# Ycblue/TransMIL-DeepGraft

Hardware: AMD Instinct MI355X
Metric: slides/sec (fwd+bwd) at N=8192 patches, d=512 (higher is better)
Workload: dtype bf16; 1 GPU; TransMIL_feat 2-class, 1 bag N=8192x512 per GPU, train step fwd+CE+bwd+allreduce+Lookahead(RAdam); execution=hipGraph replay of the whole step (one graph per resident bag), global_batch=1, seq_len=8192, parallelism=dp1, accumulate_grad_batches=1

## Files before the change

transmil_deepgraft_amd/csrc/nystrom.hip:

```cpp
#include <algorithm>
#include "common.h"
#include "nystrom_common.h"
#include "../../include/transmil_hip.h"

namespace {

template <typename T>
__global__ __launch_bounds__(256) void landmarks_kernel(const T* __restrict__ q, const T* __restrict__ k, int n,
                                                        int l, float* __restrict__ ql, float* __restrict__ kl,
                                                        T* __restrict__ ql_t, T* __restrict__ kl_t) {
  const int bh = blockIdx.x, tid = threadIdx.x, tq = tid & 3, o = ((tid >> 2) & 7) * 8;
  const int j = blockIdx.y * 8 + (tid >> 5);
  const int per = (l + 3) / 4, t0 = tq * per, t1 = min(l, t0 + per);
  const T* qp = q + ((size_t)bh * n + (size_t)j * l) * DH + o;
  const T* kp = k + ((size_t)bh * n + (size_t)j * l) * DH + o;
  float sq[8] = {0.f, 0.f, 0.f, 0.f, 0.f, 0.f, 0.f, 0.f}, sk[8] = {0.f, 0.f, 0.f, 0.f, 0.f, 0.f, 0.f, 0.f};
  for (int t = t0; t < t1; t += 9) {
    vec8<T> a[9], b[9];
#pragma unroll
    for (int u = 0; u < 9; ++u) {
      const int tt = min(t + u, t1 - 1);
      a[u] = load8(qp + (size_t)tt * DH);
      b[u] = load8(kp + (size_t)tt * DH);
    }
// ... 373 lines not shown
  float* po = work;
  float* pm = po + (size_t)nkb * nbh * NL * DH;
  float* pl = pm + (size_t)nkb * nbh * NL;
  tm_allow_smem(a3_fwd_kernel, FWD_F32_SMEM);
  a3_fwd_kernel<<<dim3(nkb, nbh, 2), 256, FWD_F32_SMEM, st>>>(ql, (const float*)k, (const float*)v, n, po, pm, pl);
  TM_CHECK_LAUNCH();
  a3_combine_kernel<<<dim3(nbh, NL / 16), 256, 0, st>>>(po, pm, pl, nkb, nbh, w, lse3);
  TM_CHECK_LAUNCH();
  return 0;
}

extern "C" int tm_nys_a3_fwd_sim2(const float* ql, const float* kl, const void* k, const void* v, int nbh, int n,
                                  float* work, float* a2, void* a2s, void* stream) {
  TM_REQUIRE(n > 0 && n % NL == 0, "a3_fwd_sim2: n must be a positive multiple of 256");
  TM_REQUIRE(ql && kl && k && v && work && a2 && a2s, "a3_fwd_sim2: null operand");
  launch_a3_fwd_v2(ql, k, v, nbh, n, work, Sim2Out{kl, a2, (bf16*)a2s}, (hipStream_t)stream);
  TM_CHECK_LAUNCH();
  return 0;
}

extern "C" int tm_nys_a1_fwd(int dtype, const void* q, const void* v, const void* kl_t, const void* y_t,
                             const float* wconv, int nbh, int nh, int n, void* merged, float* lse1, void* stream) {
  TM_REQUIRE(n > 0 && n % NL == 0 && nbh % nh == 0, "a1_fwd: bad shape");
  hipStream_t st = (hipStream_t)stream;
  if (dtype == TM_BF16) {
    const int cph = n / 32;
    int wpg = std::max(1, std::min(tm_cu_count() / std::max(nbh, 1), cph));
    wpg = std::max(wpg, (cph + A1P_MAXCH - 1) / A1P_MAXCH);
    auto kern = a1_fwd_bf16_kernel<false>;
#ifdef TM_DIAG
    if (NYS_SEL == NYS_STAMP_A1_FWD) kern = a1_fwd_bf16_kernel<true>;
#endif
    tm_allow_smem(kern, A1P_BYTES);
    kern<<<dim3(wpg, nbh), 256, A1P_BYTES, st>>>((const bf16*)q, (const bf16*)v, (const bf16*)kl_t,
                                                               (const bf16*)y_t, wconv, n, nh, wpg, (bf16*)merged,
                                                               lse1);
    TM_CHECK_LAUNCH();
    return 0;
  }
  TM_REQUIRE_F32(dtype);
  constexpr size_t sm = FWD_F32_SMEM > A1_EPI_BYTES ? FWD_F32_SMEM : A1_EPI_BYTES;
  tm_allow_smem(a1_fwd_kernel, sm);
  a1_fwd_kernel<<<dim3(n / 128, nbh), 256, sm, st>>>((const float*)q, (const float*)v, (const float*)kl_t,
                                                     (const float*)y_t, wconv, n, nh, (float*)merged, lse1);
  TM_CHECK_LAUNCH();
  return 0;
}

extern "C" int tm_cast_f32(int dtype, const float* x, void* y, long long count, void* stream) {
  if (count == 0) return 0;
  TM_REQUIRE(((uintptr_t)x % 16) == 0 && ((uintptr_t)y % 16) == 0, "cast_f32: 16-B aligned buffers");
  TM_DTYPE_DISPATCH(dtype, (cast_rows_kernel<T><<<(unsigned)((count + 2047) / 2048), 256, 0, (hipStream_t)stream>>>(
                               x, (T*)y, count)));
  TM_CHECK_LAUNCH();
  return 0;
}

extern "C" long long tm_nys_conv_bwd_workspace(int nbags, int nh, int n) {
  const int r = conv_bwd_rows(nbags * nh, n);
  const long long blocks = std::max((n + 63) / 64, (n + r - 1) / r);
  return (long long)nbags * blocks * nh * TAPS * (long long)sizeof(float);
}

extern "C" int tm_nys_conv_bwd(int dtype, const void* dmerged, const void* merged, const void* v, const float* wconv,
                               int nbh, int nh, int n, void* dv, float* d1, float* work, float* dwconv,
                               tm_reduce_queue* rq, void* stream) {
  TM_REQUIRE(nbh % nh == 0 && n > 0, "conv_bwd: bad shape");
  hipStream_t st = (hipStream_t)stream;
  if (dtype == TM_BF16) {
    const int r = conv_bwd_rows(nbh, n), nblk = (n + r - 1) / r;
    tm_allow_smem(conv_bwd_mfma_kernel, CbLay::BYTES);
    conv_bwd_mfma_kernel<<<dim3(nblk, nbh), 512, CbLay::BYTES, st>>>(
        (const bf16*)dmerged, (const bf16*)merged, (const bf16*)v, wconv, n, nh, r, (bf16*)dv, d1, work);
    TM_CHECK_LAUNCH();
    return tm_splitk_reduce(work, dwconv, (nbh / nh) * nblk, (long long)nh * TAPS, 1.0f, 0, rq, stream);
  }
  TM_REQUIRE_F32(dtype);
  const int ntb = (n + 63) / 64;
  conv_bwd_kernel<<<dim3(ntb, nbh), 256, 0, st>>>((const float*)dmerged, (const float*)merged, (const float*)v, wconv,
                                                  n, nh, (float*)dv, d1, work);
  TM_CHECK_LAUNCH();
  return tm_splitk_reduce(work, dwconv, (nbh / nh) * ntb, (long long)nh * TAPS, 1.0f, 0, rq, stream);
}

namespace {
int a1_bwd_split(int nbh, int n) {
  const int cph = n / 32;
  const int w = std::min(cph, std::max(1, tm_cu_count() / std::max(nbh, 1)));
  return std::max(w, (cph + BwdLay16::MAXQ / 32 - 1) / (BwdLay16::MAXQ / 32));
}
}

extern "C" long long tm_nys_a1_bwd_workspace(int nbh, int n, int queries_per_wg) {
  const long long slabs = std::max((long long)(n / queries_per_wg), (long long)a1_bwd_split(nbh, n));
  return 2LL * slabs * nbh * NL * DH * (long long)sizeof(float);
}

namespace {
int a1_bwd_impl(int dtype, const void* q, const void* dmerged, const void* kl_t, const void* y_t, const float* lse1,
                const float* d1, int nbh, int nh, int n, int queries_per_wg, float* dq, void* dqkv, float dq_scale,
                float* work, float* dkl, float* dy, int accumulate, tm_reduce_queue* rq, void* stream);
}

extern "C" int tm_nys_a1_bwd(int dtype, const void* q, const void* dmerged, const void* kl_t, const void* y_t,
                             const float* lse1, const float* d1, int nbh, int nh, int n, int queries_per_wg,
                             float* dq, float* work, float* dkl, float* dy, int accumulate, tm_reduce_queue* rq,
                             void* stream) {
  return a1_bwd_impl(dtype, q, dmerged, kl_t, y_t, lse1, d1, nbh, nh, n, queries_per_wg, dq, nullptr, 0.f, work, dkl,
                     dy, accumulate, rq, stream);
}

extern "C" int tm_nys_a1_bwd_dqkv(const void* q, const void* dmerged, const void* kl_t, const void* y_t,
                                  const float* lse1, const float* d1, int nbh, int nh, int n, void* dqkv,
                                  float dq_scale, float* work, float* dkl, float* dy, tm_reduce_queue* rq,
                                  void* stream) {
  TM_REQUIRE(dqkv && ((uintptr_t)dqkv % 16) == 0 && nbh % nh == 0, "a1_bwd_dqkv: dqkv");
  return a1_bwd_impl(TM_BF16, q, dmerged, kl_t, y_t, lse1, d1, nbh, nh, n, 256, nullptr, dqkv, dq_scale, work, dkl,
                     dy, 0, rq, stream);
}

namespace {
int a1_bwd_impl(int dtype, const void* q, const void* dmerged, const void* kl_t, const void* y_t, const float* lse1,
                const float* d1, int nbh, int nh, int n, int queries_per_wg, float* dq, void* dqkv, float dq_scale,
                float* work, float* dkl, float* dy, int accumulate, tm_reduce_queue* rq, void* stream) {
  TM_REQUIRE(queries_per_wg % 32 == 0 && n % queries_per_wg == 0, "a1_bwd: queries_per_wg must divide n, x32");
  TM_REQUIRE(dtype != TM_BF16 || queries_per_wg <= NL, "a1_bwd: queries_per_wg must be <= 256 in bf16 mode");
  const bool split = dtype == TM_BF16;
  TM_REQUIRE(!dqkv || split, "a1_bwd_dqkv: the bf16 split kernel only");
  const int nqc = split ? a1_bwd_split(nbh, n) : n / queries_per_wg;
  BwdArgs a{};
  a.q = q; a.q_bag = (long long)nh * n * DH; a.q_head = (long long)n * DH; a.q_row = DH;
  a.dO = dmerged; a.o_bag = (long long)n * nh * DH; a.o_head = DH; a.o_row = nh * DH;
  a.k = kl_t; a.k_bag = (long long)nh * NL * DH; a.k_head = (long long)NL * DH;
  a.v = y_t; a.v_bag = a.k_bag; a.v_head = a.k_head;
  a.lse = lse1; a.lse_bh = n; a.dd = d1; a.dd_bh = n;
  a.dq = dq; a.dq_bh = (long long)n * DH;
  a.dqkv = dqkv; a.dq_scale = dq_scale;
  float* slab_k = work;
  float* slab_v = work + (size_t)nqc * nbh * NL * DH;
  a.dk = slab_k; a.dk_bh = (long long)NL * DH;
  a.dv = slab_v; a.dv_bh = (long long)NL * DH;
  a.slab_stride = (long long)nbh * NL * DH;
  a.nh = nh; a.n_queries_per_wg = queries_per_wg; a.n_key_rows = NL;
  hipStream_t st = (hipStream_t)stream;
  if (split) {
    a.q_total = n;
    a.slab_bf16 = 1;
    auto kern = attn_bwd_bf16_kernel<MODE_A1>;
#ifdef TM_DIAG
    if (NYS_SEL == NYS_STAMP_A1_BWD) kern = attn_bwd_bf16_kernel<MODE_A1, 8, 1>;
    if (NYS_SEL == NYS_STAMP_A1_BWD_CHUNK) kern = attn_bwd_bf16_kernel<MODE_A1, 8, 2>;
#endif
    tm_allow_smem(kern, BwdLay16::BYTES);
    kern<<<dim3(nqc, nbh), 512, BwdLay16::BYTES, st>>>(a);
  } else {
    TM_REQUIRE_F32(dtype);
    tm_allow_smem(attn_bwd_kernel<MODE_A1>, BwdLayF32::BYTES);
    attn_bwd_kernel<MODE_A1><<<dim3(nqc, nbh), 512, BwdLayF32::BYTES, st>>>(a);
  }
  TM_CHECK_LAUNCH();
  const long long cnt = (long long)nbh * NL * DH;
  const int sdt = a.slab_bf16 ? TM_BF16 : TM_F32;
  int rc = tm_splitk_reduce_typed(slab_k, sdt, dkl, nqc, cnt, 1.0f, accumulate, rq, stream);
  if (rc) return rc;
  return tm_splitk_reduce_typed(slab_v, sdt, dy, nqc, cnt, 1.0f, 0, rq, stream);
}
}

namespace {
struct A3Split { int wpg, nw; };
A3Split a3_bwd_split(int nbh, int n) {
  const int units = n / 32;
  const int w = std::max(1, std::min(units, tm_cu_count() / std::max(nbh, 1)));
  const int per = (units + w - 1) / w;
  if (per <= 8) return {w, 8};
  if (per == 9) return {w, 9};
  return {(units + 7) / 8, 8};
}

void launch_a3_bwd_bf16(BwdArgs& a, int nbh, int n, hipStream_t st, int& slabs) {
  const A3Split sp = a3_bwd_split(nbh, n);
  a.q_total = n;
  slabs = sp.wpg;
  if (sp.nw == 9) {
    auto kern = attn_bwd_bf16_kernel<MODE_A3, 9>;
#ifdef TM_DIAG
    if (NYS_SEL == NYS_STAMP_A3_BWD) kern = attn_bwd_bf16_kernel<MODE_A3, 9, 1>;
    if (NYS_SEL == NYS_STAMP_A3_BWD_CHUNK) kern = attn_bwd_bf16_kernel<MODE_A3, 9, 2>;
#endif
    tm_allow_smem(kern, BwdLay9::BYTES);
    kern<<<dim3(sp.wpg, nbh), 576, BwdLay9::BYTES, st>>>(a);
  } else {
    tm_allow_smem(attn_bwd_bf16_kernel<MODE_A3, 8>, BwdLay16::BYTES);
    attn_bwd_bf16_kernel<MODE_A3, 8><<<dim3(sp.wpg, nbh), 512, BwdLay16::BYTES, st>>>(a);
  }
}
}

extern "C" long long tm_nys_a3_bwd_workspace(int nbh, int n) {
  const long long slabs = std::max((long long)(n / NL), (long long)a3_bwd_split(nbh, n).wpg);
  return slabs * nbh * NL * DH * (long long)sizeof(float);
}

extern "C" int tm_nys_a3_bwd(int dtype, const void* ql_t, const void* dw_t, const void* k, const void* v,
                             const float* lse3, const float* d3, int nbh, int nh, int n, float* dk, float* dv,
                             float* work, float* dql, int accumulate, tm_reduce_queue* rq, void* stream) {
  TM_REQUIRE(n % NL == 0, "a3_bwd: n must be a multiple of 256");
  const int nkb = n / NL;
  BwdArgs a{};
  a.q = ql_t; a.q_bag = (long long)nh * NL * DH; a.q_head = (long long)NL * DH; a.q_row = DH;
  a.dO = dw_t; a.o_bag = a.q_bag; a.o_head = a.q_head; a.o_row = DH;
  a.k = k; a.k_bag = (long long)nh * n * DH; a.k_head = (long long)n * DH;
  a.v = v; a.v_bag = a.k_bag; a.v_head = a.k_head;
  a.lse = lse3; a.lse_bh = NL; a.dd = d3; a.dd2 = d3 + (size_t)nbh * NL; a.dd_bh = NL;
  a.dq = work; a.dq_bh = (long long)NL * DH;
  a.slab_stride = (long long)nbh * NL * DH;
  a.dk = dk; a.dk_bh = (long long)n * DH;
  a.dv = dv; a.dv_bh = (long long)n * DH;
  a.nh = nh; a.n_queries_per_wg = NL; a.n_key_rows = n;
  hipStream_t st = (hipStream_t)stream;
  int slabs = nkb;
  if (dtype == TM_BF16) {
    launch_a3_bwd_bf16(a, nbh, n, st, slabs);
  } else {
    TM_REQUIRE_F32(dtype);
    tm_allow_smem(attn_bwd_kernel<MODE_A3>, BwdLayF32::BYTES);
    attn_bwd_kernel<MODE_A3><<<dim3(nkb, nbh), 512, BwdLayF32::BYTES, st>>>(a);
  }
  TM_CHECK_LAUNCH();
  return tm_splitk_reduce(work, dql, slabs, (long long)nbh * NL * DH, 1.0f, accumulate, rq, stream);
}

extern "C" int tm_nys_a3_bwd_fused(const void* ql_t, const void* dw_t, const void* k, const void* v,
                                   const float* lse3, const float* d3, int nbh, int nh, int n, const void* dv_conv,
                                   int dv_lo, int dv_hi, const float* dkl, float* work, float* dql, void* dqkv,
                                   tm_reduce_queue* rq, void* stream) {
  TM_REQUIRE(n % NL == 0 && nbh % nh == 0, "a3_bwd_fused: n must be a multiple of 256");
  TM_REQUIRE(dv_conv && dkl && dqkv, "a3_bwd_fused: null operand");
  const int nkb = n / NL;
  BwdArgs a{};
  a.q = ql_t; a.q_bag = (long long)nh * NL * DH; a.q_head = (long long)NL * DH; a.q_row = DH;
  a.dO = dw_t; a.o_bag = a.q_bag; a.o_head = a.q_head; a.o_row = DH;
  a.k = k; a.k_bag = (long long)nh * n * DH; a.k_head = (long long)n * DH;
  a.v = v; a.v_bag = a.k_bag; a.v_head = a.k_head;
  a.lse = lse3; a.lse_bh = NL; a.dd = d3; a.dd2 = d3 + (size_t)nbh * NL; a.dd_bh = NL;
  a.dq = work; a.dq_bh = (long long)NL * DH;
  a.slab_stride = (long long)nbh * NL * DH;
  a.dv = (float*)dv_conv; a.dv_bh = (long long)n * DH;
  a.nh = nh; a.n_queries_per_wg = NL; a.n_key_rows = n;
  a.dqkv = dqkv; a.dkl = dkl; a.l = n / NL; a.inv_l = 1.0f / (float)(n / NL);
  a.dv_lo = dv_lo; a.dv_hi = dv_hi;
  hipStream_t st = (hipStream_t)stream;
  int slabs = nkb;
  a.slab_bf16 = 1;
  launch_a3_bwd_bf16(a, nbh, n, st, slabs);
  TM_CHECK_LAUNCH();
  if (!dql) return 0;
  return tm_splitk_reduce_typed(work, TM_BF16, dql, slabs, (long long)nbh * NL * DH, 1.0f, 0, rq, stream);
}

extern "C" int tm_nys_a3_bwd_slabs(int nbh, int n) { return a3_bwd_split(nbh, n).wpg; }

extern "C" int tm_nys_assemble_q_slab(int dtype, const float* dq, int dq_row, const float* dql, const void* slab,
                                      int slabs, int nbags, int nh, int n, float scale, void* dqkv, void* stream) {
  TM_REQUIRE(n > 0 && n % NL == 0 && nh > 0 && nh <= 8 && slabs > 0, "assemble_q_slab: bad shape");
  TM_REQUIRE(dq && dql && slab && dqkv, "assemble_q_slab: null operand");
  TM_DTYPE_DISPATCH(dtype, (assemble_q_slab_kernel<T><<<dim3(NL, nbags), AQ_THREADS, 0, (hipStream_t)stream>>>(
                               dq, dq_row, dql, (const bf16*)slab, slabs, (long long)nbags * nh * NL * DH, n, n / NL,
                               nh, scale, (T*)dqkv)));
  TM_CHECK_LAUNCH();
  return 0;
}

extern "C" int tm_nys_assemble_q_slab_inplace(const float* dql, const void* slab, int slabs, int nbags, int nh, int n,
                                              float scale, void* dqkv, void* stream) {
  TM_REQUIRE(n > 0 && n % NL == 0 && nh > 0 && nh <= 8 && slabs > 0, "assemble_q_slab_inplace: bad shape");
  TM_REQUIRE(dql && slab && dqkv && ((uintptr_t)dqkv % 16) == 0, "assemble_q_slab_inplace: null / misaligned operand");
  assemble_q_slab_kernel<bf16, true><<<dim3(NL, nbags), AQ_THREADS, 0, (hipStream_t)stream>>>(
      nullptr, -1, dql, (const bf16*)slab, slabs, (long long)nbags * nh * NL * DH, n, n / NL, nh, scale, (bf16*)dqkv);
  TM_CHECK_LAUNCH();
  return 0;
}

extern "C" int tm_nys_assemble_dqkv(int dtype, const float* dq, const float* dql, const float* dk, const float* dkl,
                                    const float* dv, int nbags, int nh, int n, float scale, void* dqkv,
                                    void* stream) {
  TM_REQUIRE(n % NL == 0, "assemble_dqkv: n must be a multiple of 256");
  const long long items = (long long)n * 3 * nh * DH / 8;
  TM_DTYPE_DISPATCH(dtype, (assemble_dqkv_kernel<T><<<dim3((unsigned)((items + 255) / 256), nbags), 256, 0,
                                                       (hipStream_t)stream>>>(
                               dq, dql, dk, dkl, dv, n, n / NL, nh, scale, (T*)dqkv)));
  TM_CHECK_LAUNCH();
  return 0;
}
```

transmil_deepgraft_amd/csrc/nystrom_bf16.h:

```cpp
#pragma once
#include <algorithm>
#include <type_traits>
#include "nystrom_common.h"
#include "a3_combine.h"

namespace {

constexpr int A1P_WAVES = 4;
constexpr int A1P_MAXCH = 9;
constexpr int A1P_WROWS = A1P_MAXCH * 32 + 32;
constexpr int A1P_OROW = DH + 8;
constexpr size_t A1P_KS = (size_t)NL * Lay<bf16>::KROW * 2;
constexpr size_t A1P_VT = (size_t)NL * Lay<bf16>::VROW * 2;
constexpr size_t A1P_WIN = (size_t)A1P_WROWS * DH * 2;
constexpr size_t A1P_OST = (size_t)32 * A1P_OROW * 2;
constexpr size_t A1P_WIN_OFF = A1P_KS + A1P_VT;
constexpr size_t A1P_OST_OFF = A1P_WIN_OFF + A1P_WIN;
constexpr size_t A1P_BAND_OFF = A1P_OST_OFF + A1P_WAVES * A1P_OST;
constexpr size_t A1P_TAPS_OFF = A1P_BAND_OFF + 4 * 64 * 16;
constexpr size_t A1P_BYTES = A1P_TAPS_OFF + 128 * sizeof(float);

__device__ unsigned long long g_a1_stamps[512 * 8 * 8];
template <bool STAMP>
TM_DEV void a1p_stamp(int slot, int wave) {
// ... 420 lines not shown
  const int k = kb + 8 * (g >> 1) + q;
  typedef __attribute__((address_space(3))) bf16x4 lds_v4;
  const bf16x4 lo = __builtin_amdgcn_ds_read_tr16_b64_v4bf16((lds_v4*)(S + k * ldr + m));
  const bf16x4 hi = __builtin_amdgcn_ds_read_tr16_b64_v4bf16((lds_v4*)(S + (k + 4) * ldr + m));
  return (bf16x8){lo[0], lo[1], lo[2], lo[3], hi[0], hi[1], hi[2], hi[3]};
}

__global__ __launch_bounds__(512) void conv_bwd_mfma_kernel(const bf16* __restrict__ dmerged,
                                                            const bf16* __restrict__ merged,
                                                            const bf16* __restrict__ v,
                                                            const float* __restrict__ wconv, int n, int nh, int R,
                                                            bf16* __restrict__ dv, float* __restrict__ d1,
                                                            float* __restrict__ dw_part) {
  extern __shared__ __attribute__((aligned(16))) char smem[];
  bf16* dos = (bf16*)(smem + CbLay::DO_OFF);
  bf16* vws = (bf16*)(smem + CbLay::V_OFF);
  float* ws = (float*)(smem + CbLay::W_OFF);
  float* csum = (float*)(smem + CbLay::CS_OFF);
  const int tid = threadIdx.x, lane = tid & 63, wave = tid >> 6, r32 = lane & 31, h = lane >> 5;
  const int bh = blockIdx.y, blk = blockIdx.x, nblk = gridDim.x;
  const int head = bh % nh, bag = bh / nh, ld = nh * DH;
  const int t0 = blk * R;
  const int rows = min(R, n - t0);
  const bf16* dob = dmerged + (size_t)bag * n * ld + head * DH;
  const bf16* ob = merged + (size_t)bag * n * ld + head * DH;
  const bf16* vb = v + (size_t)bh * n * DH;
  constexpr int PW = CB_WIN * 8 / 512;
  bf16x8 ca[PW], cb[PW];
#pragma unroll
  for (int j = 0; j < PW; ++j) {
    const int i = tid + 512 * j, w = i >> 3, d0 = (i & 7) * 8, t = t0 - HALF + w;
    const bool ok = t >= 0 && t < n && w < rows + 2 * HALF;
    const int tc = ok ? t : 0;
    ca[j] = load8(dob + (size_t)tc * ld + d0);
    cb[j] = load8(vb + (size_t)tc * DH + d0);
    if (!ok) { ca[j] = (bf16x8){}; cb[j] = (bf16x8){}; }
  }
  if (tid < TAPS) ws[tid] = wconv[head * TAPS + tid];
#pragma unroll
  for (int j = 0; j < PW; ++j) {
    const int i = tid + 512 * j, w = i >> 3, d0 = (i & 7) * 8;
    *(bf16x8*)(dos + w * CB_ROW + d0) = ca[j];
    *(bf16x8*)(vws + w * CB_ROW + d0) = cb[j];
  }
  __syncthreads();
  bf16x8 th[4], tl[4];
#pragma unroll
  for (int st = 0; st < 4; ++st) {
#pragma unroll
    for (int j = 0; j < 8; ++j) {
      const int tau = r32 + 32 - (16 * st + 8 * h + j);
      const float wv = (tau >= 0 && tau < TAPS) ? ws[tau] : 0.f;
      const bf16 hi = (bf16)wv;
      th[st][j] = hi;
      tl[st][j] = (bf16)(wv - (float)hi);
    }
  }
  float* stg = (float*)(smem + CbLay::ST_OFF) + wave * 32 * CB_ST;
  constexpr int NTK = (TAPS + 1) / 2;
  float csl[NTK];
#pragma unroll
  for (int k = 0; k < NTK; ++k) csl[k] = 0.f;
  const int ntile = (rows + 31) / 32;
#pragma unroll 1
  for (int i = wave; i < ntile; i += 8) {
    f32x16 sa = (f32x16){}, sb = (f32x16){};
#pragma unroll
    for (int st = 0; st < 4; ++st) {
      const bf16x8 a = *(const bf16x8*)(dos + (32 * i + HALF + r32) * CB_ROW + 16 * st + 8 * h);
      const bf16x8 ba = *(const bf16x8*)(vws + (32 * i + r32) * CB_ROW + 16 * st + 8 * h);
      const bf16x8 bb = *(const bf16x8*)(vws + (32 * i + 32 + r32) * CB_ROW + 16 * st + 8 * h);
      mma16(sa, a, ba);
      mma16(sb, a, bb);
    }
#pragma unroll
    for (int reg = 0; reg < 16; ++reg) {
      const int row = acc_row(reg, h);
      stg[row * CB_ST + r32] = sa[reg];
      stg[row * CB_ST + 32 + r32] = sb[reg];
    }
    __builtin_amdgcn_fence(__ATOMIC_RELEASE, "wavefront");
    __builtin_amdgcn_wave_barrier();
    __builtin_amdgcn_fence(__ATOMIC_ACQUIRE, "wavefront");
    const int lr = 32 * i + r32;
    const bool rv = lr < rows;
    float wc = 0.f, dd = 0.f;
#pragma unroll
    for (int k = 0; k < NTK; ++k) {
      const int tau = h + 2 * k;
      if (tau < TAPS) {
        const float c = stg[r32 * CB_ST + r32 + tau];
        if (rv) { csl[k] += c; wc = fmaf(ws[tau], c, wc); }
      }
    }
    if (rv) {
      const bf16* orow = ob + (size_t)(t0 + lr) * ld + 32 * h;
      const bf16* grow = dos + (lr + HALF) * CB_ROW + 32 * h;
#pragma unroll
      for (int q = 0; q < 4; ++q) {
        const bf16x8 o8 = load8(orow + 8 * q), g8 = *(const bf16x8*)(grow + 8 * q);
#pragma unroll
        for (int e = 0; e < 8; ++e) dd = fmaf((float)g8[e], (float)o8[e], dd);
      }
    }
    float tot = dd - wc;
    tot += __shfl_xor(tot, 32, 64);
    if (rv && h == 0) d1[(size_t)bh * n + t0 + lr] = tot;
    const bf16* dwin = dos + 32 * i * CB_ROW;
#pragma unroll
    for (int dt = 0; dt < 2; ++dt) {
      f32x16 acc = (f32x16){};
#pragma unroll
      for (int st = 0; st < 4; ++st) {
        const bf16x8 b = frag_tr_rows(dwin, CB_ROW, dt * 32, 16 * st, lane);
        mma16(acc, th[st], b);
        mma16(acc, tl[st], b);
      }
#pragma unroll
      for (int reg = 0; reg < 16; ++reg) {
        const int l2 = 32 * i + acc_row(reg, h);
        if (l2 < rows) dv[((size_t)bh * n + t0 + l2) * DH + dt * 32 + r32] = (bf16)acc[reg];
      }
    }
    __builtin_amdgcn_wave_barrier();
  }
#pragma unroll
  for (int k = 0; k < NTK; ++k) {
    float x = csl[k];
#pragma unroll
    for (int o = 1; o < 32; o <<= 1) x += __shfl_xor(x, o, 64);
    const int tau = h + 2 * k;
    if (r32 == 0 && tau < TAPS) csum[wave * 36 + tau] = x;
  }
  __syncthreads();
  if (tid < TAPS) {
    float sum = 0.f;
#pragma unroll
    for (int w = 0; w < 8; ++w) sum += csum[w * 36 + tid];
    dw_part[((size_t)bag * nblk + blk) * (nh * TAPS) + head * TAPS + tid] = sum;
  }
}

enum NysSel { NYS_AUTO = 0, NYS_STAMP_A1_FWD, NYS_STAMP_A3_FWD, NYS_STAMP_A1_BWD, NYS_STAMP_A1_BWD_CHUNK,
              NYS_STAMP_A3_BWD, NYS_STAMP_A3_BWD_CHUNK };
#ifdef TM_DIAG
int g_nys_sel = NYS_AUTO;
#endif
#define NYS_SEL TM_DIAG_VAR(g_nys_sel)

template <int NW, int MQ>
struct BwdLayT {
  static constexpr int MAXQ = MQ;
  static constexpr int NK = 32 * NW;
  static constexpr int KT_ROW = NK + 8, DS_ROW = NK + 8, QROW = DH + 8;
  static constexpr size_t KT_OFF = 0;
  static constexpr size_t DS_OFF = KT_OFF + DH * KT_ROW * 2;
  static constexpr size_t QS_OFF = DS_OFF + 32 * DS_ROW * 2;
  static constexpr size_t OS_OFF = QS_OFF + MAXQ * QROW * 2;
  static constexpr size_t XC_OFF = OS_OFF + MAXQ * QROW * 2;
  static constexpr size_t LS_OFF = XC_OFF + 6 * 1024 * 4;
  static constexpr size_t MAIN = LS_OFF + 2 * MAXQ * 4;
  static constexpr size_t EPI = (size_t)NK * 68 * 4;
  static constexpr size_t BYTES = MAIN > EPI ? MAIN : EPI;
};
using BwdLay16 = BwdLayT<8, 288>;
using BwdLay9 = BwdLayT<9, 256>;
static_assert(BwdLay9::BYTES <= 160 * 1024 && BwdLay16::BYTES <= 160 * 1024, "bf16 backward layout exceeds the CU's LDS");

template <int R>
TM_DEV bf16x8 frag_tr_rows(const bf16* S, int mb, int kb, int lane) {
  const int g = lane >> 4, q = (lane & 15) >> 2, p = lane & 3;
  const int m = mb + (g & 1) * 16 + 4 * p;
  const int k = kb + 4 * (g >> 1) + q;
  typedef __attribute__((address_space(3))) bf16x4 lds_v4;
  const bf16x4 lo = __builtin_amdgcn_ds_read_tr16_b64_v4bf16((lds_v4*)(S + k * R + m));
  const bf16x4 hi = __builtin_amdgcn_ds_read_tr16_b64_v4bf16((lds_v4*)(S + (k + 8) * R + m));
  return (bf16x8){lo[0], lo[1], lo[2], lo[3], hi[0], hi[1], hi[2], hi[3]};
}
TM_DEV bf16x8 frag_tr_acc(const bf16* S, int mb, int kb, int lane) { return frag_tr_rows<BwdLay16::QROW>(S, mb, kb, lane); }

template <int MODE, int NW = 8, int ST = 0>
__global__ __launch_bounds__(64 * NW) void attn_bwd_bf16_kernel(BwdArgs a) {
  using LY = std::conditional_t<NW == 9, BwdLay9, BwdLay16>;
  static_assert(NW == 8 || (NW == 9 && MODE == MODE_A3), "9-wave form: A3 even split only");
  constexpr int NT = 64 * NW;
  constexpr int KT_ROW = LY::KT_ROW, DS_ROW = LY::DS_ROW, QROW = LY::QROW;
  extern __shared__ __attribute__((aligned(16))) char smem[];
  bf16* kt_s = (bf16*)(smem + LY::KT_OFF);
  bf16* ds_s = (bf16*)(smem + LY::DS_OFF);
  bf16* qs = (bf16*)(smem + LY::QS_OFF);
  bf16* os = (bf16*)(smem + LY::OS_OFF);
  float* lse_s = (float*)(smem + LY::LS_OFF);
  float* dd_s = lse_s + LY::MAXQ;
  float* stage = (float*)smem;

  const int tid = threadIdx.x, lane = tid & 63, wave = tid >> 6, r = lane & 31, h = lane >> 5;
  const int blk = blockIdx.x, bh = blockIdx.y, nh = a.nh;
  auto stamp = [&](int slot) { if (ST == 1 && wave < 8) a1p_stamp<ST != 0>(slot, wave); };
  auto cstamp = [&](int c0, int slot) { if (ST == 2 && c0 == 64 && wave < 8) a1p_stamp<ST != 0>(slot, wave); };
  stamp(0);
  int key0 = (MODE == MODE_A3) ? blk * NL : 0;
  int nunits = 8;
  if (MODE == MODE_A3 && a.q_total > 0) {
    const int upk = a.n_key_rows / 32;
    const int u0 = (int)((long long)blk * upk / gridDim.x), u1 = (int)((long long)(blk + 1) * upk / gridDim.x);
    key0 = 32 * u0;
    nunits = u1 - u0;
  }
  const int nk = 32 * nunits;
  const bool active = wave < nunits;
  int q_begin = (MODE == MODE_A1) ? blk * a.n_queries_per_wg : 0;
  int q_count = a.n_queries_per_wg;
  if (MODE == MODE_A1 && a.q_total > 0) {
    const int cph = a.q_total / 32;
    const int c0 = (int)((long long)blk * cph / gridDim.x), c1 = (int)((long long)(blk + 1) * cph / gridDim.x);
    q_begin = 32 * c0;
    q_count = 32 * (c1 - c0);
  }

  const bf16* Q = (const bf16*)a.q + hoff(bh, nh, a.q_bag, a.q_head) + (size_t)q_begin * a.q_row;
  const bf16* dO = (const bf16*)a.dO + hoff(bh, nh, a.o_bag, a.o_head) + (size_t)q_begin * a.o_row;
  const bf16* K = (const bf16*)a.k + hoff(bh, nh, a.k_bag, a.k_head) + (size_t)key0 * DH;
  const bf16* V = (const bf16*)a.v + hoff(bh, nh, a.v_bag, a.v_head) + (size_t)key0 * DH;
  const float* lse = a.lse + bh * a.lse_bh + q_begin;
  const float* dd = a.dd + bh * a.dd_bh + q_begin;
  const float* dd2 = a.dd2 ? a.dd2 + bh * a.dd_bh + q_begin : nullptr;

  constexpr int QP = (LY::MAXQ * 8 + NT - 1) / NT;
  const int mykey = wave * 32;
  bf16x8 qr[QP], orow[QP], kf[4], vf[4];
#pragma unroll
  for (int j = 0; j < QP; ++j) {
    const int c = tid + NT * j;
    const int qq = min(c >> 3, q_count - 1);
    qr[j] = load8(Q + (size_t)qq * a.q_row + (c & 7) * 8);
    orow[j] = load8(dO + (size_t)qq * a.o_row + (c & 7) * 8);
  }
  const int kfr = min(mykey + r, nk - 1);
#pragma unroll
  for (int st = 0; st < 4; ++st) {
    kf[st] = load8(K + (size_t)kfr * DH + st * 16 + 8 * h);
    vf[st] = load8(V + (size_t)kfr * DH + st * 16 + 8 * h);
  }
  float lsev = 0.f, ddv = 0.f;
  if (tid < LY::MAXQ) {
    const int qq = min(tid, q_count - 1);
    lsev = lse[qq];
    ddv = dd[qq] + (dd2 ? dd2[qq] : 0.f);
  }
  __builtin_amdgcn_sched_barrier(0);
  stamp(1);
#pragma unroll
  for (int st = 0; st < 4; ++st) {
#pragma unroll
    for (int e = 0; e < 8; ++e) kt_s[(st * 16 + 8 * h + e) * KT_ROW + mykey + r] = kf[st][e];
  }
#pragma unroll
  for (int j = 0; j < QP; ++j) {
    const int c = tid + NT * j, row = c >> 3, d0 = (c & 7) * 8;
    if (row < LY::MAXQ) {
      *(bf16x8*)(qs + row * QROW + d0) = qr[j];
      *(bf16x8*)(os + row * QROW + d0) = orow[j];
    }
  }
  if (tid < LY::MAXQ) {
    lse_s[tid] = lsev;
    dd_s[tid] = ddv;
  }
  __syncthreads();
  stamp(2);

  f32x16 dvt[2], dkt[2];
#pragma unroll
  for (int i = 0; i < 2; ++i) { dvt[i] = (f32x16){}; dkt[i] = (f32x16){}; }

#pragma unroll 1
  for (int c0 = 0; c0 < q_count; c0 += 32) {
    f32x16 s = (f32x16){}, dp = (f32x16){};
    cstamp(c0, 0);
    if (active) {
#pragma unroll
      for (int st = 0; st < 4; ++st) {
        const bf16x8 qa_f = *(const bf16x8*)(qs + (c0 + r) * QROW + st * 16 + 8 * h);
        const bf16x8 oa_f = *(const bf16x8*)(os + (c0 + r) * QROW + st * 16 + 8 * h);
        mma16(s, qa_f, kf[st]);
        mma16(dp, oa_f, vf[st]);
      }
#pragma unroll
      for (int i = 0; i < 16; ++i) {
        const int qq = c0 + acc_row(i, h);
        const float p = __expf(s[i] - lse_s[qq]);
        s[i] = p;
        dp[i] = p * (dp[i] - dd_s[qq]);
      }
#pragma unroll
      for (int sp = 0; sp < 2; ++sp) {
        const bf16x8 bp = acc_as_operand<bf16>(s, sp);
        const bf16x8 bs = acc_as_operand<bf16>(dp, sp);
#pragma unroll
        for (int dt = 0; dt < 2; ++dt) {
          const bf16x8 ao = frag_tr_acc(os + c0 * QROW, dt * 32, 16 * sp, lane);
          const bf16x8 aq = frag_tr_acc(qs + c0 * QROW, dt * 32, 16 * sp, lane);
          mma16(dvt[dt], ao, bp);
          mma16(dkt[dt], aq, bs);
        }
      }
    }
    cstamp(c0, 1);
    __syncthreads();
    cstamp(c0, 2);
#pragma unroll
    for (int i = 0; i < 16; ++i) ds_s[acc_row(i, h) * DS_ROW + mykey + r] = from_f<bf16>(dp[i]);
    __syncthreads();
    cstamp(c0, 3);
    {
      constexpr int W0 = NW == 9 ? 1 : 0;
      if (wave == W0 || wave == W0 + 1) {
        const int dtq = wave - W0;
        f32x16 acc = (f32x16){};
        constexpr int NS = 2 * NW;
        const bf16* da = ds_s + r * DS_ROW + 8 * h;
        const bf16* kb = kt_s + (dtq * 32 + r) * KT_ROW + 8 * h;
        bf16x8 fa[4], fb[4];
#pragma unroll
        for (int st = 0; st < 2; ++st) { fa[st] = load8(da + st * 16); fb[st] = load8(kb + st * 16); }
#pragma unroll
        for (int st = 0; st < NS; st += 2) {
#pragma unroll
          for (int u = 2; u < 4; ++u)
            if (st + u < NS) { fa[(st + u) & 3] = load8(da + (st + u) * 16); fb[(st + u) & 3] = load8(kb + (st + u) * 16); }
          __builtin_amdgcn_sched_barrier(0);
          mma16(acc, fa[st & 3], fb[st & 3]);
          if (st + 1 < NS) mma16(acc, fa[(st + 1) & 3], fb[(st + 1) & 3]);
          __builtin_amdgcn_sched_barrier(0);
        }
        cstamp(c0, 4);
        if (MODE == MODE_A1 && a.dqkv) {
          const int bag = bh / nh, hh = bh % nh, ld = 3 * nh * DH;
          bf16* qo = (bf16*)a.dqkv + ((size_t)bag * a.q_total + q_begin + c0) * ld + hh * DH + dtq * 32 + r;
#pragma unroll
          for (int i = 0; i < 16; ++i) qo[(size_t)acc_row(i, h) * ld] = (bf16)(a.dq_scale * acc[i]);
        } else if (MODE == MODE_A3 && a.slab_bf16) {
          bf16* dst = (bf16*)a.dq + (size_t)blk * a.slab_stride + bh * a.dq_bh + (size_t)(q_begin + c0) * DH + dtq * 32 + r;
#pragma unroll
          for (int i = 0; i < 16; ++i) dst[(size_t)acc_row(i, h) * DH] = (bf16)acc[i];
        } else {
          float* dst = MODE == MODE_A1 ? a.dq + bh * a.dq_bh : a.dq + (size_t)blk * a.slab_stride + bh * a.dq_bh;
          dst += (size_t)(q_begin + c0) * DH + dtq * 32 + r;
#pragma unroll
          for (int i = 0; i < 16; ++i) dst[(size_t)acc_row(i, h) * DH] = acc[i];
        }
        cstamp(c0, 5);
      }
    }
    if (c0 == 0) stamp(3);
    if (c0 == 96) stamp(4);
  }
  stamp(5);
  __syncthreads();
  if (MODE == MODE_A3 && a.dqkv) {
    constexpr int IT = (LY::NK * DH / 8 + NT - 1) / NT;
    static_assert(2 * LY::NK * 68 * 4 <= LY::BYTES, "fused A3 epilogue: two staged tiles exceed the layout");
    const int bag = bh / nh, hh = bh % nh, inner = nh * DH;
    bf16* outk = (bf16*)a.dqkv + ((size_t)bag * a.n_key_rows + key0) * 3 * inner + inner + hh * DH;
    bf16* outv = outk + inner;
    const bf16* dvc = (const bf16*)a.dv + bh * a.dv_bh + (size_t)key0 * DH;
    const float* dkl = a.dkl + (size_t)bh * NL * DH;
    f32x4 av[IT][2], ak[IT][2];
#pragma unroll
    for (int it = 0; it < IT; ++it) {
      const int i = tid + NT * it, key = i >> 3, d8 = (i & 7) * 8;
      const bool valid = key < nk;
      const bool vw = valid && key0 + key >= a.dv_lo && key0 + key < a.dv_hi;
      const bf16x8 pv = vw ? *(const bf16x8*)(dvc + (size_t)min(key, nk - 1) * DH + d8) : (bf16x8){};
      av[it][0] = (f32x4){(float)pv[0], (float)pv[1], (float)pv[2], (float)pv[3]};
      av[it][1] = (f32x4){(float)pv[4], (float)pv[5], (float)pv[6], (float)pv[7]};
    }
    float* stage_k = stage + LY::NK * 68;
#pragma unroll
    for (int dt = 0; dt < 2; ++dt)
#pragma unroll
      for (int g4 = 0; g4 < 4; ++g4) {
        const int o = (mykey + r) * 68 + dt * 32 + 8 * g4 + 4 * h;
        *(f32x4*)(stage + o) = (f32x4){dvt[dt][4 * g4], dvt[dt][4 * g4 + 1], dvt[dt][4 * g4 + 2], dvt[dt][4 * g4 + 3]};
        *(f32x4*)(stage_k + o) = (f32x4){dkt[dt][4 * g4], dkt[dt][4 * g4 + 1], dkt[dt][4 * g4 + 2], dkt[dt][4 * g4 + 3]};
      }
#pragma unroll
    for (int it = 0; it < IT; ++it) {
      const int i = tid + NT * it, key = min(i >> 3, nk - 1), d8 = (i & 7) * 8;
      const float* pk = dkl + (size_t)((key0 + key) / a.l) * DH + d8;
      ak[it][0] = *(const f32x4*)pk;
      ak[it][1] = *(const f32x4*)(pk + 4);
    }
    __syncthreads();
    const float il = a.inv_l;
#pragma unroll
    for (int it = 0; it < IT; ++it) {
      const int i = tid + NT * it, key = i >> 3, d8 = (i & 7) * 8;
      if (key >= nk) continue;
      const float* sv = stage + key * 68 + d8;
      const float* sk = stage_k + key * 68 + d8;
      const f32x4 v0 = *(const f32x4*)sv + av[it][0], v1 = *(const f32x4*)(sv + 4) + av[it][1];
      const f32x4 k0 = *(const f32x4*)sk + ak[it][0] * il, k1 = *(const f32x4*)(sk + 4) + ak[it][1] * il;
      *(bf16x8*)(outv + (size_t)key * 3 * inner + d8) =
          (bf16x8){(bf16)v0[0], (bf16)v0[1], (bf16)v0[2], (bf16)v0[3], (bf16)v1[0], (bf16)v1[1], (bf16)v1[2], (bf16)v1[3]};
      *(bf16x8*)(outk + (size_t)key * 3 * inner + d8) =
          (bf16x8){(bf16)k0[0], (bf16)k0[1], (bf16)k0[2], (bf16)k0[3], (bf16)k1[0], (bf16)k1[1], (bf16)k1[2], (bf16)k1[3]};
    }
    stamp(6);
    return;
  }
#pragma unroll
  for (int which = 0; which < 2; ++which) {
#pragma unroll
    for (int dt = 0; dt < 2; ++dt) {
      const f32x16& accv = which == 0 ? dvt[dt] : dkt[dt];
#pragma unroll
      for (int g4 = 0; g4 < 4; ++g4)
        *(f32x4*)(stage + (mykey + r) * 68 + dt * 32 + 8 * g4 + 4 * h) =
            (f32x4){accv[4 * g4], accv[4 * g4 + 1], accv[4 * g4 + 2], accv[4 * g4 + 3]};
    }
    __syncthreads();
    if (MODE == MODE_A1 && a.slab_bf16) {
      bf16* dstb = (bf16*)(which == 0 ? a.dv : a.dk) + (size_t)blk * a.slab_stride + bh * (which == 0 ? a.dv_bh : a.dk_bh);
      for (int i = tid; i < nk * DH / 4; i += NT) {
        const int key = i >> 4, d4 = (i & 15) * 4;
        const f32x4 val = *(const f32x4*)(stage + key * 68 + d4);
        *(bf16x4*)(dstb + (size_t)key * DH + d4) = (bf16x4){(bf16)val[0], (bf16)val[1], (bf16)val[2], (bf16)val[3]};
      }
      __syncthreads();
      continue;
    }
    float* dst;
    bool add = false;
    if (MODE == MODE_A3) {
      dst = (which == 0 ? a.dv + bh * a.dv_bh : a.dk + bh * a.dk_bh) + (size_t)key0 * DH;
      add = (which == 0);
    } else {
      dst = (which == 0 ? a.dv : a.dk) + (size_t)blk * a.slab_stride + bh * (which == 0 ? a.dv_bh : a.dk_bh);
    }
    for (int i = tid; i < nk * DH / 4; i += NT) {
      const int key = i >> 4, d4 = (i & 15) * 4;
      f32x4 val = *(const f32x4*)(stage + key * 68 + d4);
      float* p = dst + (size_t)key * DH + d4;
      if (add) val += *(const f32x4*)p;
      *(f32x4*)p = val;
    }
    __syncthreads();
  }
  stamp(6);
}

}
```

Before: 944.0 slides/sec.

## Warp-specialize attention backward with dedicated dQ waves and double-buffered dS

The bf16 Nystrom attention backward kernel gains two extra waves per workgroup that only compute dQ = dS·K. They read a double-buffered, key-major dS tile through transposed LDS reads. The key waves write dS into alternating buffers and need one barrier per chunk instead of two, so the dQ MMA for chunk c overlaps the key waves' dV/dK work for chunk c+1 rather than stalling all waves on two MMA-busy waves. The change also vectorizes the lse/delta loads and drops the unused XC scratch region. In exchange, threads per block and register pressure under the new launch bounds go up, the dS LDS footprint doubles, and the EPI stage size now accounts for both dV and dK.

```diff
diff --git a/transmil_deepgraft_amd/csrc/nystrom.hip b/transmil_deepgraft_amd/csrc/nystrom.hip
--- a/transmil_deepgraft_amd/csrc/nystrom.hip
+++ b/transmil_deepgraft_amd/csrc/nystrom.hip
@@ -549,7 +549,7 @@
     if (NYS_SEL == NYS_STAMP_A1_BWD_CHUNK) kern = attn_bwd_bf16_kernel<MODE_A1, 8, 2>;
 #endif
     tm_allow_smem(kern, BwdLay16::BYTES);
-    kern<<<dim3(nqc, nbh), 512, BwdLay16::BYTES, st>>>(a);
+    kern<<<dim3(nqc, nbh), 640, BwdLay16::BYTES, st>>>(a);
   } else {
     TM_REQUIRE_F32(dtype);
     tm_allow_smem(attn_bwd_kernel<MODE_A1>, BwdLayF32::BYTES);
@@ -586,10 +586,10 @@
     if (NYS_SEL == NYS_STAMP_A3_BWD_CHUNK) kern = attn_bwd_bf16_kernel<MODE_A3, 9, 2>;
 #endif
     tm_allow_smem(kern, BwdLay9::BYTES);
-    kern<<<dim3(sp.wpg, nbh), 576, BwdLay9::BYTES, st>>>(a);
+    kern<<<dim3(sp.wpg, nbh), 704, BwdLay9::BYTES, st>>>(a);
   } else {
     tm_allow_smem(attn_bwd_bf16_kernel<MODE_A3, 8>, BwdLay16::BYTES);
-    attn_bwd_bf16_kernel<MODE_A3, 8><<<dim3(sp.wpg, nbh), 512, BwdLay16::BYTES, st>>>(a);
+    attn_bwd_bf16_kernel<MODE_A3, 8><<<dim3(sp.wpg, nbh), 640, BwdLay16::BYTES, st>>>(a);
   }
 }
 }
diff --git a/transmil_deepgraft_amd/csrc/nystrom_bf16.h b/transmil_deepgraft_amd/csrc/nystrom_bf16.h
--- a/transmil_deepgraft_amd/csrc/nystrom_bf16.h
+++ b/transmil_deepgraft_amd/csrc/nystrom_bf16.h
@@ -596,15 +596,16 @@
 struct BwdLayT {
   static constexpr int MAXQ = MQ;
   static constexpr int NK = 32 * NW;
-  static constexpr int KT_ROW = NK + 8, DS_ROW = NK + 8, QROW = DH + 8;
+  static constexpr int KT_ROW = NK + 8, QROW = DH + 8;
+  static constexpr int DS_ROW = 36;
+  static constexpr int DS_BUF = NK * DS_ROW;
   static constexpr size_t KT_OFF = 0;
   static constexpr size_t DS_OFF = KT_OFF + DH * KT_ROW * 2;
-  static constexpr size_t QS_OFF = DS_OFF + 32 * DS_ROW * 2;
+  static constexpr size_t QS_OFF = DS_OFF + 2 * DS_BUF * 2;
   static constexpr size_t OS_OFF = QS_OFF + MAXQ * QROW * 2;
-  static constexpr size_t XC_OFF = OS_OFF + MAXQ * QROW * 2;
-  static constexpr size_t LS_OFF = XC_OFF + 6 * 1024 * 4;
+  static constexpr size_t LS_OFF = OS_OFF + MAXQ * QROW * 2;
   static constexpr size_t MAIN = LS_OFF + 2 * MAXQ * 4;
-  static constexpr size_t EPI = (size_t)NK * 68 * 4;
+  static constexpr size_t EPI = 2 * (size_t)NK * 68 * 4;
   static constexpr size_t BYTES = MAIN > EPI ? MAIN : EPI;
 };
 using BwdLay16 = BwdLayT<8, 288>;
@@ -622,12 +623,22 @@
   return (bf16x8){lo[0], lo[1], lo[2], lo[3], hi[0], hi[1], hi[2], hi[3]};
 }
 TM_DEV bf16x8 frag_tr_acc(const bf16* S, int mb, int kb, int lane) { return frag_tr_rows<BwdLay16::QROW>(S, mb, kb, lane); }
+template <int R>
+TM_DEV bf16x8 frag_tr_nat(const bf16* S, int kb, int lane) {
+  const int g = lane >> 4, q = (lane & 15) >> 2, p = lane & 3;
+  const int m = (g & 1) * 16 + 4 * p;
+  const int k = kb + 8 * (g >> 1) + q;
+  typedef __attribute__((address_space(3))) bf16x4 lds_v4;
+  const bf16x4 lo = __builtin_amdgcn_ds_read_tr16_b64_v4bf16((lds_v4*)(S + k * R + m));
+  const bf16x4 hi = __builtin_amdgcn_ds_read_tr16_b64_v4bf16((lds_v4*)(S + (k + 4) * R + m));
+  return (bf16x8){lo[0], lo[1], lo[2], lo[3], hi[0], hi[1], hi[2], hi[3]};
+}
 
 template <int MODE, int NW = 8, int ST = 0>
-__global__ __launch_bounds__(64 * NW) void attn_bwd_bf16_kernel(BwdArgs a) {
+__global__ __launch_bounds__(64 * (NW + 2)) void attn_bwd_bf16_kernel(BwdArgs a) {
   using LY = std::conditional_t<NW == 9, BwdLay9, BwdLay16>;
   static_assert(NW == 8 || (NW == 9 && MODE == MODE_A3), "9-wave form: A3 even split only");
-  constexpr int NT = 64 * NW;
+  constexpr int NT = 64 * (NW + 2);
   constexpr int KT_ROW = LY::KT_ROW, DS_ROW = LY::DS_ROW, QROW = LY::QROW;
   extern __shared__ __attribute__((aligned(16))) char smem[];
   bf16* kt_s = (bf16*)(smem + LY::KT_OFF);
@@ -638,10 +649,14 @@
   float* dd_s = lse_s + LY::MAXQ;
   float* stage = (float*)smem;
 
-  const int tid = threadIdx.x, lane = tid & 63, wave = tid >> 6, r = lane & 31, h = lane >> 5;
+  const int tid = threadIdx.x, lane = tid & 63, r = lane & 31, h = lane >> 5;
+  const int wave = __builtin_amdgcn_readfirstlane(tid >> 6);
   const int blk = blockIdx.x, bh = blockIdx.y, nh = a.nh;
-  auto stamp = [&](int slot) { if (ST == 1 && wave < 8) a1p_stamp<ST != 0>(slot, wave); };
-  auto cstamp = [&](int c0, int slot) { if (ST == 2 && c0 == 64 && wave < 8) a1p_stamp<ST != 0>(slot, wave); };
+  const bool keyw = wave < NW;
+  const bool stamped = wave < 6 || !keyw;
+  const int srow = keyw ? wave : 6 + wave - NW;
+  auto stamp = [&](int slot) { if (ST == 1 && stamped) a1p_stamp<ST != 0>(slot, srow); };
+  auto cstamp = [&](int c0, int slot) { if (ST == 2 && c0 == 64 && stamped) a1p_stamp<ST != 0>(slot, srow); };
   stamp(0);
   int key0 = (MODE == MODE_A3) ? blk * NL : 0;
   int nunits = 8;
@@ -681,10 +696,12 @@
     orow[j] = load8(dO + (size_t)qq * a.o_row + (c & 7) * 8);
   }
   const int kfr = min(mykey + r, nk - 1);
-#pragma unroll
-  for (int st = 0; st < 4; ++st) {
-    kf[st] = load8(K + (size_t)kfr * DH + st * 16 + 8 * h);
-    vf[st] = load8(V + (size_t)kfr * DH + st * 16 + 8 * h);
+  if (keyw) {
+#pragma unroll
+    for (int st = 0; st < 4; ++st) {
+      kf[st] = load8(K + (size_t)kfr * DH + st * 16 + 8 * h);
+      vf[st] = load8(V + (size_t)kfr * DH + st * 16 + 8 * h);
+    }
   }
   float lsev = 0.f, ddv = 0.f;
   if (tid < LY::MAXQ) {
@@ -694,10 +711,12 @@
   }
   __builtin_amdgcn_sched_barrier(0);
   stamp(1);
-#pragma unroll
-  for (int st = 0; st < 4; ++st) {
-#pragma unroll
-    for (int e = 0; e < 8; ++e) kt_s[(st * 16 + 8 * h + e) * KT_ROW + mykey + r] = kf[st][e];
+  if (keyw) {
+#pragma unroll
+    for (int st = 0; st < 4; ++st) {
+#pragma unroll
+      for (int e = 0; e < 8; ++e) kt_s[(st * 16 + 8 * h + e) * KT_ROW + mykey + r] = kf[st][e];
+    }
   }
 #pragma unroll
   for (int j = 0; j < QP; ++j) {
@@ -718,87 +737,102 @@
 #pragma unroll
   for (int i = 0; i < 2; ++i) { dvt[i] = (f32x16){}; dkt[i] = (f32x16){}; }
 
+  const int nchunk = q_count / 32;
+  if (keyw) {
 #pragma unroll 1
-  for (int c0 = 0; c0 < q_count; c0 += 32) {
-    f32x16 s = (f32x16){}, dp = (f32x16){};
-    cstamp(c0, 0);
-    if (active) {
-#pragma unroll
-      for (int st = 0; st < 4; ++st) {
-        const bf16x8 qa_f = *(const bf16x8*)(qs + (c0 + r) * QROW + st * 16 + 8 * h);
-        const bf16x8 oa_f = *(const bf16x8*)(os + (c0 + r) * QROW + st * 16 + 8 * h);
-        mma16(s, qa_f, kf[st]);
-        mma16(dp, oa_f, vf[st]);
-      }
-#pragma unroll
-      for (int i = 0; i < 16; ++i) {
-        const int qq = c0 + acc_row(i, h);
-        const float p = __expf(s[i] - lse_s[qq]);
-        s[i] = p;
-        dp[i] = p * (dp[i] - dd_s[qq]);
-      }
-#pragma unroll
-      for (int sp = 0; sp < 2; ++sp) {
-        const bf16x8 bp = acc_as_operand<bf16>(s, sp);
-        const bf16x8 bs = acc_as_operand<bf16>(dp, sp);
-#pragma unroll
-        for (int dt = 0; dt < 2; ++dt) {
-          const bf16x8 ao = frag_tr_acc(os + c0 * QROW, dt * 32, 16 * sp, lane);
-          const bf16x8 aq = frag_tr_acc(qs + c0 * QROW, dt * 32, 16 * sp, lane);
-          mma16(dvt[dt], ao, bp);
-          mma16(dkt[dt], aq, bs);
+    for (int c = 0; c < nchunk; ++c) {
+      const int c0 = 32 * c;
+      f32x16 s = (f32x16){}, dp = (f32x16){};
+      cstamp(c0, 0);
+      if (active) {
+#pragma unroll
+        for (int st = 0; st < 4; ++st) {
+          const bf16x8 qa_f = *(const bf16x8*)(qs + (c0 + r) * QROW + st * 16 + 8 * h);
+          const bf16x8 oa_f = *(const bf16x8*)(os + (c0 + r) * QROW + st * 16 + 8 * h);
+          mma16(s, qa_f, kf[st]);
+          mma16(dp, oa_f, vf[st]);
         }
-      }
-    }
-    cstamp(c0, 1);
-    __syncthreads();
-    cstamp(c0, 2);
-#pragma unroll
-    for (int i = 0; i < 16; ++i) ds_s[acc_row(i, h) * DS_ROW + mykey + r] = from_f<bf16>(dp[i]);
-    __syncthreads();
-    cstamp(c0, 3);
-    {
-      constexpr int W0 = NW == 9 ? 1 : 0;
-      if (wave == W0 || wave == W0 + 1) {
-        const int dtq = wave - W0;
-        f32x16 acc = (f32x16){};
-        constexpr int NS = 2 * NW;
-        const bf16* da = ds_s + r * DS_ROW + 8 * h;
-        const bf16* kb = kt_s + (dtq * 32 + r) * KT_ROW + 8 * h;
-        bf16x8 fa[4], fb[4];
-#pragma unroll
-        for (int st = 0; st < 2; ++st) { fa[st] = load8(da + st * 16); fb[st] = load8(kb + st * 16); }
-#pragma unroll
-        for (int st = 0; st < NS; st += 2) {
-#pragma unroll
-          for (int u = 2; u < 4; ++u)
-            if (st + u < NS) { fa[(st + u) & 3] = load8(da + (st + u) * 16); fb[(st + u) & 3] = load8(kb + (st + u) * 16); }
-          __builtin_amdgcn_sched_barrier(0);
-          mma16(acc, fa[st & 3], fb[st & 3]);
-          if (st + 1 < NS) mma16(acc, fa[(st + 1) & 3], fb[(st + 1) & 3]);
-          __builtin_amdgcn_sched_barrier(0);
+#pragma unroll
+        for (int g4 = 0; g4 < 4; ++g4) {
+          const f32x4 l4 = *(const f32x4*)(lse_s + c0 + 8 * g4 + 4 * h);
+          const f32x4 d4 = *(const f32x4*)(dd_s + c0 + 8 * g4 + 4 * h);
+#pragma unroll
+          for (int e = 0; e < 4; ++e) {
+            const int i = 4 * g4 + e;
+            const float p = __expf(s[i] - l4[e]);
+            s[i] = p;
+            dp[i] = p * (dp[i] - d4[e]);
+          }
         }
-        cstamp(c0, 4);
-        if (MODE == MODE_A1 && a.dqkv) {
-          const int bag = bh / nh, hh = bh % nh, ld = 3 * nh * DH;
-          bf16* qo = (bf16*)a.dqkv + ((size_t)bag * a.q_total + q_begin + c0) * ld + hh * DH + dtq * 32 + r;
-#pragma unroll
-          for (int i = 0; i < 16; ++i) qo[(size_t)acc_row(i, h) * ld] = (bf16)(a.dq_scale * acc[i]);
-        } else if (MODE == MODE_A3 && a.slab_bf16) {
-          bf16* dst = (bf16*)a.dq + (size_t)blk * a.slab_stride + bh * a.dq_bh + (size_t)(q_begin + c0) * DH + dtq * 32 + r;
-#pragma unroll
-          for (int i = 0; i < 16; ++i) dst[(size_t)acc_row(i, h) * DH] = (bf16)acc[i];
-        } else {
-          float* dst = MODE == MODE_A1 ? a.dq + bh * a.dq_bh : a.dq + (size_t)blk * a.slab_stride + bh * a.dq_bh;
-          dst += (size_t)(q_begin + c0) * DH + dtq * 32 + r;
-#pragma unroll
-          for (int i = 0; i < 16; ++i) dst[(size_t)acc_row(i, h) * DH] = acc[i];
+#pragma unroll
+        for (int sp = 0; sp < 2; ++sp) {
+          const bf16x8 bp = acc_as_operand<bf16>(s, sp);
+          const bf16x8 bs = acc_as_operand<bf16>(dp, sp);
+#pragma unroll
+          for (int dt = 0; dt < 2; ++dt) {
+            const bf16x8 ao = frag_tr_acc(os + c0 * QROW, dt * 32, 16 * sp, lane);
+            const bf16x8 aq = frag_tr_acc(qs + c0 * QROW, dt * 32, 16 * sp, lane);
+            mma16(dvt[dt], ao, bp);
+            mma16(dkt[dt], aq, bs);
+          }
         }
-        cstamp(c0, 5);
-      }
-    }
-    if (c0 == 0) stamp(3);
-    if (c0 == 96) stamp(4);
+      }
+      cstamp(c0, 1);
+      bf16* dsw = ds_s + (c & 1) * LY::DS_BUF + (mykey + r) * DS_ROW + 4 * h;
+#pragma unroll
+      for (int g4 = 0; g4 < 4; ++g4)
+        *(bf16x4*)(dsw + 8 * g4) = (bf16x4){from_f<bf16>(dp[4 * g4]), from_f<bf16>(dp[4 * g4 + 1]),
+                                            from_f<bf16>(dp[4 * g4 + 2]), from_f<bf16>(dp[4 * g4 + 3])};
+      cstamp(c0, 2);
+      __syncthreads();
+      cstamp(c0, 3);
+      if (c == 0) stamp(3);
+      if (c == 3) stamp(4);
+    }
+  } else {
+#pragma unroll 1
+    for (int c = 0; c < nchunk; ++c) {
+      __syncthreads();
+      const int c0 = 32 * c, dtq = wave - NW;
+      cstamp(c0 - 32, 3);
+      if (c == 0) stamp(3);
+      if (c == 3) stamp(4);
+      cstamp(c0, 0);
+      f32x16 acc = (f32x16){};
+      constexpr int NS = 2 * NW;
+      const bf16* da = ds_s + (c & 1) * LY::DS_BUF;
+      const bf16* kb = kt_s + (dtq * 32 + r) * KT_ROW + 8 * h;
+      bf16x8 fa[4], fb[4];
+#pragma unroll
+      for (int st = 0; st < 2; ++st) { fa[st] = frag_tr_nat<DS_ROW>(da, st * 16, lane); fb[st] = load8(kb + st * 16); }
+#pragma unroll
+      for (int st = 0; st < NS; st += 2) {
+#pragma unroll
+        for (int u = 2; u < 4; ++u)
+          if (st + u < NS) { fa[(st + u) & 3] = frag_tr_nat<DS_ROW>(da, (st + u) * 16, lane); fb[(st + u) & 3] = load8(kb + (st + u) * 16); }
+        __builtin_amdgcn_sched_barrier(0);
+        mma16(acc, fa[st & 3], fb[st & 3]);
+        if (st + 1 < NS) mma16(acc, fa[(st + 1) & 3], fb[(st + 1) & 3]);
+        __builtin_amdgcn_sched_barrier(0);
+      }
+      cstamp(c0, 1);
+      if (MODE == MODE_A1 && a.dqkv) {
+        const int bag = bh / nh, hh = bh % nh, ld = 3 * nh * DH;
+        bf16* qo = (bf16*)a.dqkv + ((size_t)bag * a.q_total + q_begin + c0) * ld + hh * DH + dtq * 32 + r;
+#pragma unroll
+        for (int i = 0; i < 16; ++i) qo[(size_t)acc_row(i, h) * ld] = (bf16)(a.dq_scale * acc[i]);
+      } else if (MODE == MODE_A3 && a.slab_bf16) {
+        bf16* dst = (bf16*)a.dq + (size_t)blk * a.slab_stride + bh * a.dq_bh + (size_t)(q_begin + c0) * DH + dtq * 32 + r;
+#pragma unroll
+        for (int i = 0; i < 16; ++i) dst[(size_t)acc_row(i, h) * DH] = (bf16)acc[i];
+      } else {
+        float* dst = MODE == MODE_A1 ? a.dq + bh * a.dq_bh : a.dq + (size_t)blk * a.slab_stride + bh * a.dq_bh;
+        dst += (size_t)(q_begin + c0) * DH + dtq * 32 + r;
+#pragma unroll
+        for (int i = 0; i < 16; ++i) dst[(size_t)acc_row(i, h) * DH] = acc[i];
+      }
+      cstamp(c0, 2);
+    }
   }
   stamp(5);
   __syncthreads();
@@ -821,14 +855,16 @@
       av[it][1] = (f32x4){(float)pv[4], (float)pv[5], (float)pv[6], (float)pv[7]};
     }
     float* stage_k = stage + LY::NK * 68;
-#pragma unroll
-    for (int dt = 0; dt < 2; ++dt)
-#pragma unroll
-      for (int g4 = 0; g4 < 4; ++g4) {
-        const int o = (mykey + r) * 68 + dt * 32 + 8 * g4 + 4 * h;
-        *(f32x4*)(stage + o) = (f32x4){dvt[dt][4 * g4], dvt[dt][4 * g4 + 1], dvt[dt][4 * g4 + 2], dvt[dt][4 * g4 + 3]};
-        *(f32x4*)(stage_k + o) = (f32x4){dkt[dt][4 * g4], dkt[dt][4 * g4 + 1], dkt[dt][4 * g4 + 2], dkt[dt][4 * g4 + 3]};
-      }
+    if (keyw) {
+#pragma unroll
+      for (int dt = 0; dt < 2; ++dt)
+#pragma unroll
+        for (int g4 = 0; g4 < 4; ++g4) {
+          const int o = (mykey + r) * 68 + dt * 32 + 8 * g4 + 4 * h;
+          *(f32x4*)(stage + o) = (f32x4){dvt[dt][4 * g4], dvt[dt][4 * g4 + 1], dvt[dt][4 * g4 + 2], dvt[dt][4 * g4 + 3]};
+          *(f32x4*)(stage_k + o) = (f32x4){dkt[dt][4 * g4], dkt[dt][4 * g4 + 1], dkt[dt][4 * g4 + 2], dkt[dt][4 * g4 + 3]};
+        }
+    }
 #pragma unroll
     for (int it = 0; it < IT; ++it) {
       const int i = tid + NT * it, key = min(i >> 3, nk - 1), d8 = (i & 7) * 8;
@@ -856,13 +892,15 @@
   }
 #pragma unroll
   for (int which = 0; which < 2; ++which) {
-#pragma unroll
-    for (int dt = 0; dt < 2; ++dt) {
-      const f32x16& accv = which == 0 ? dvt[dt] : dkt[dt];
-#pragma unroll
-      for (int g4 = 0; g4 < 4; ++g4)
-        *(f32x4*)(stage + (mykey + r) * 68 + dt * 32 + 8 * g4 + 4 * h) =
-            (f32x4){accv[4 * g4], accv[4 * g4 + 1], accv[4 * g4 + 2], accv[4 * g4 + 3]};
+    if (keyw) {
+#pragma unroll
+      for (int dt = 0; dt < 2; ++dt) {
+        const f32x16& accv = which == 0 ? dvt[dt] : dkt[dt];
+#pragma unroll
+        for (int g4 = 0; g4 < 4; ++g4)
+          *(f32x4*)(stage + (mykey + r) * 68 + dt * 32 + 8 * g4 + 4 * h) =
+              (f32x4){accv[4 * g4], accv[4 * g4 + 1], accv[4 * g4 + 2], accv[4 * g4 + 3]};
+      }
     }
     __syncthreads();
     if (MODE == MODE_A1 && a.slab_bf16) {
```

Result: no change. 948.9 slides/sec (median of 6 runs) (+0.5%).
